# richox/orz

Hardware: AMD Instinct MI355X
Metric: orz -l1 encode throughput (enwik8-shaped text, 100 MB, one 16 MiB block in flight) (higher is better)
Workload: dtype u8

## Files before the change

### orz_amd/csrc/backend_hip.h

```cpp
#pragma once
#include <hip/hip_runtime.h>

#include <cxxabi.h>

#include <chrono>
#include <condition_variable>
#include <algorithm>
#include <atomic>
#include <cstring>
#include <map>
#include <mutex>
#include <rocprim/rocprim.hpp>
#include <stdexcept>
#include <string>
#include <type_traits>
#include <vector>

#include "orz_kernels.h"
#include "orz_parse.h"
#include "orz_symrank.h"

namespace orz {

#define ORZ_HIP_CHECK(expr)                                                                              \
    do {                                                                                                 \
        hipError_t e_ = (expr);                                                                          \
        if (e_ != hipSuccess)                                                                            \
            throw std::runtime_error(std::string("HIP error: ") + hipGetErrorString(e_) + " at " #expr); \
    } while (0)

template <class F>
__global__ __launch_bounds__(256) void orz_thread_kernel(F f, size_t n) {
    size_t tid = (size_t)blockIdx.x * blockDim.x + threadIdx.x;
    if (tid < n) f(tid);
}

#if defined(ORZ_EVAL_WAVES)
template <class F>
__global__ __launch_bounds__(256) __attribute__((amdgpu_waves_per_eu(ORZ_EVAL_WAVES, ORZ_EVAL_WAVES))) void orz_thread_kernel_occ(F f, size_t n) {
    size_t tid = (size_t)blockIdx.x * blockDim.x + threadIdx.x;
    if (tid < n) f(tid);
}
#endif

struct DevWave {
    uint8_t* lds_;
    __device__ __forceinline__ uint32_t lane() const { return threadIdx.x; }
    __device__ __forceinline__ uint32_t block() const { return blockIdx.x; }
    __device__ __forceinline__ uint8_t* lds() const { return lds_; }
    __device__ __forceinline__ uint64_t ballot(bool p) const { return __ballot(p); }
    __device__ __forceinline__ void sync() const { __syncthreads(); }
    __device__ __forceinline__ uint32_t bcast(uint32_t v, uint32_t src) const {
        return (uint32_t)__builtin_amdgcn_readlane((int)v, (int)src);
    }
    __device__ __forceinline__ uint32_t shfl(uint32_t v, uint32_t src) const { return (uint32_t)__shfl((int)v, (int)src, 64); }
    __device__ __forceinline__ uint64_t bcast64(uint64_t v, uint32_t src) const {
        const uint32_t lo = (uint32_t)__builtin_amdgcn_readlane((int)(uint32_t)v, (int)src);
        const uint32_t hi = (uint32_t)__builtin_amdgcn_readlane((int)(uint32_t)(v >> 32), (int)src);
        return (uint64_t)lo | ((uint64_t)hi << 32);
    }
    __device__ __forceinline__ unsigned long long clock() const { return __builtin_amdgcn_s_memtime(); }
    __device__ __forceinline__ unsigned long long wallclock() const { return __builtin_amdgcn_s_memrealtime(); }
};
template <class K>
__global__ __launch_bounds__(64) void orz_wave_kernel(K k) {
    extern __shared__ __attribute__((aligned(16))) uint8_t orz_dyn_lds[];
    DevWave w{orz_dyn_lds};
    k(w);
}

template <class K>
__global__ __launch_bounds__(1024) void orz_group_kernel(K k, bool use_lds) {
    extern __shared__ __attribute__((aligned(16))) uint8_t orz_dyn_lds[];
    for (uint32_t ph = 0; ph < K::kPhases; ph++) {
        if (ph) {
            __threadfence_block();
            __syncthreads();
        }
        k.phase(ph, threadIdx.x, blockDim.x, orz_dyn_lds, use_lds);
    }
}

__global__ __launch_bounds__(256) void orz_rank_kernel(RankArgs a, uint32_t nchunks, uint32_t nvblk) {
    __shared__ uint32_t rows[(kRankChunk + 1) * 256];
    auto sync = [] __device__() { __syncthreads(); };
    if (blockIdx.x < nchunks) rank_chunk(a, blockIdx.x, threadIdx.x, rows, sync);
    else if (blockIdx.x < nchunks + nvblk)
        rebuild_summaries(a.vbits, a.v1, a.v2, a.nvwords, blockIdx.x - nchunks, threadIdx.x, (uint64_t*)rows, sync);
    else
        rebuild_summaries(a.kbits, a.k1, a.k2, a.nkwords, blockIdx.x - nchunks - nvblk, threadIdx.x, (uint64_t*)rows, sync);
}


struct FastEval;

class ParseTokens {
   public:
    static ParseTokens& of(int device) {
        static ParseTokens t[64];
        return t[device & 63];
    }
    void acquire() {
        if (!limit()) return;
        std::unique_lock<std::mutex> lk(m_);
        cv_.wait(lk, [&] { return busy_ < limit(); });
        busy_++;
    }
    void release() {
        if (!limit()) return;
        { std::lock_guard<std::mutex> lk(m_); busy_--; }
        cv_.notify_one();
    }
    static int limit() {
        static const int n = getenv("ORZ_PARSE_TOKENS") ? atoi(getenv("ORZ_PARSE_TOKENS")) : 0;
        return n;
    }

   private:
    std::mutex m_;
    std::condition_variable cv_;
    int busy_ = 0;
// ... 232 lines not shown
    double now() {
        return std::chrono::duration<double>(std::chrono::steady_clock::now().time_since_epoch()).count();
    }
    struct Bracket {
        HipBackend& be;
        bool on;
        Bracket(HipBackend& b, int id) : be(b), on(b.profile_ && !b.capturing_) {
            if (on) be.named_begin(id);
        }
        ~Bracket() {
            if (on) be.named_end();
        }
    };
    template <class F>
    void launch(size_t n, const F& f) {
        if (!n) return;
        Bracket br(*this, profile_ ? KernelNames::of<F>() : 0);
        const unsigned grid = (unsigned)((n + 255) / 256);
#if defined(ORZ_EVAL_WAVES)
        if constexpr (std::is_same<F, FastEval>::value) {
            hipLaunchKernelGGL(orz_thread_kernel_occ<F>, dim3(grid), dim3(256), 0, stream_, f, n);
            ORZ_HIP_CHECK(hipGetLastError());
            return;
        }
#endif
        hipLaunchKernelGGL(orz_thread_kernel<F>, dim3(grid), dim3(256), 0, stream_, f, n);
        ORZ_HIP_CHECK(hipGetLastError());
    }
    template <auto Kernel>
    hipError_t big_lds(int bytes) {
        static std::atomic<int> done[64];
        std::atomic<int>* d = device_ >= 0 && device_ < 64 ? &done[device_] : nullptr;
        if (d) {
            const int v = d->load(std::memory_order_acquire);
            if (v) return (hipError_t)(v - 1);
        }
        int cur = -1;
        ORZ_HIP_CHECK(hipGetDevice(&cur));
        if (cur != device_) ORZ_HIP_CHECK(hipSetDevice(device_));
        const hipError_t e = hipFuncSetAttribute(reinterpret_cast<const void*>(Kernel), hipFuncAttributeMaxDynamicSharedMemorySize, bytes);
        if (cur != device_) ORZ_HIP_CHECK(hipSetDevice(cur));
        if (d) d->store(1 + (int)e, std::memory_order_release);
        return e;
    }
    template <class K>
    void launch_waves(size_t nblocks, const K& k, size_t lds_bytes) {
        if (!nblocks) return;
        Bracket br(*this, profile_ ? KernelNames::of<K>() : 0);
        if (lds_bytes > 64 * 1024) {
            const hipError_t big = big_lds<&orz_wave_kernel<K>>(160 * 1024 - 256);
            if (big != hipSuccess) throw std::runtime_error(std::string("hipFuncSetAttribute(MaxDynamicSharedMemorySize): ") + hipGetErrorString(big));
        }
        hipLaunchKernelGGL(orz_wave_kernel<K>, dim3((unsigned)nblocks), dim3(64), lds_bytes, stream_, k);
        ORZ_HIP_CHECK(hipGetLastError());
    }
    template <class K>
    void launch_group(const K& k) {
        Bracket br(*this, profile_ ? KernelNames::of<K>() : 0);
        size_t lds = k.lds_bytes();
        const bool big_ok = big_lds<&orz_group_kernel<K>>((int)K::kLdsMax) == hipSuccess;
        if (lds > 64 * 1024 && !big_ok) lds = 0;
        hipLaunchKernelGGL(orz_group_kernel<K>, dim3(1), dim3(1024), lds, stream_, k, lds != 0);
        ORZ_HIP_CHECK(hipGetLastError());
    }
    void huffbuild(const HuffBuild& f) {
        if (f.nchunks) launch_waves((size_t)f.nchunks * 3, HuffWave{f}, HuffWave::lds_bytes());
    }
    void rank(const RankArgs& a, uint32_t nchunks) {
        const uint32_t nvblk = (a.nvwords + 4095) / 4096, nkblk = (a.nkwords + 4095) / 4096;
        hipLaunchKernelGGL(orz_rank_kernel, dim3(nchunks + nvblk + nkblk), dim3(256), 0, stream_, a, nchunks, nvblk);
        ORZ_HIP_CHECK(hipGetLastError());
    }
    void sort_pairs_u32(const uint32_t* kin, uint32_t* kout, const uint32_t* vin, uint32_t* vout, size_t n, int bits) {
        if (n == 0) return;
        Bracket br(*this, profile_ ? KernelNames::lib("(radix sort, pairs)") : 0);
        size_t sz = tmp_bytes_;
        ORZ_HIP_CHECK(rocprim::radix_sort_pairs(tmp_, sz, kin, kout, vin, vout, n, 0, (unsigned)bits, stream_));
    }
    void sort_by_ctx(const uint16_t* ctx, uint16_t* ctx_sorted, uint32_t* perm, size_t n) {
        if (n == 0) return;
        Bracket br(*this, profile_ ? KernelNames::lib("(radix sort, items by context)") : 0);
        size_t sz = tmp_bytes_;
        ORZ_HIP_CHECK(rocprim::radix_sort_pairs(tmp_, sz, ctx, ctx_sorted, rocprim::counting_iterator<uint32_t>(0), perm, n, 0, 9, stream_));
    }
    const uint64_t* sort_u64(uint64_t* a, uint64_t* b, size_t n, int bits, int begin_bit = 0) {
        if (n == 0) return a;
        Bracket br(*this, profile_ ? KernelNames::lib("(radix sort, 64-bit keys)") : 0);
        size_t sz = tmp_bytes_;
        ORZ_HIP_CHECK(rocprim::radix_sort_keys(tmp_, sz, a, b, n, (unsigned)begin_bit, (unsigned)bits, stream_));
        return b;
    }
    void exclusive_scan_u32(const uint32_t* in, uint32_t* out, size_t n) {
        if (n == 0) return;
        Bracket br(*this, profile_ ? KernelNames::lib("(scan)") : 0);
        size_t sz = tmp_bytes_;
        ORZ_HIP_CHECK(rocprim::exclusive_scan(tmp_, sz, in, out, 0u, n, rocprim::plus<uint32_t>(), stream_));
    }
    void inclusive_max_scan_u32(const uint32_t* in, uint32_t* out, size_t n) {
        if (n == 0) return;
        Bracket br(*this, profile_ ? KernelNames::lib("(scan, running maximum)") : 0);
        size_t sz = tmp_bytes_;
        ORZ_HIP_CHECK(rocprim::inclusive_scan(tmp_, sz, in, out, n, rocprim::maximum<uint32_t>(), stream_));
    }
    static constexpr int kTimedSlots = 4;
    void timed_begin(int slot = 0) {
        if (!timing_ || capturing_ || ((slot == 0 || slot == 3) && !profile_)) return;
// ... 199 lines not shown
```

### orz_amd/csrc/orz_fast.h

```cpp
#pragma once
#include "orz_kernels.h"
#include "orz_parse.h"

namespace orz {

#if !defined(__HIPCC__)
inline unsigned long long g_far_stats[4] = {0, 0, 0, 0};
#endif

constexpr uint32_t kSub = 4096;
constexpr uint32_t kSeg64 = 64;
constexpr uint32_t kNSub = kNewMax / kSub + 2;
constexpr uint32_t kEntries = 240;

constexpr uint32_t kFastK = 32;
constexpr uint32_t kHistSub = (kPre + 1) / kSub;
constexpr uint32_t kRingMargin = 4;
constexpr uint32_t kFastTile = 262144;
constexpr uint32_t kFastRounds = 4;
constexpr uint32_t kSettledTile = 393216;
constexpr uint32_t kSettledTileDeep = 262144;
constexpr uint32_t kSettledRounds = 3;

struct FastArgs {
// ... 989 lines not shown
                    const uint32_t d = p < a.len ? fast_decide(p, a.len, e[q], e[q + 1], e[q + 2]) : 0;
                    tyw |= (uint64_t)(d & 0xff) << (8 * q);
                    nlw |= (uint64_t)((d >> 8) & 0xff) << (8 * q);
                }
                if ((x >> 10) == part) {
                    if (x + 8 <= clen) {
                        *reinterpret_cast<uint64_t*>(a.ty + i0) = tyw;
                        *reinterpret_cast<uint64_t*>(a.nl + i0) = nlw;
                    } else {
                        for (uint32_t q = 0; x + q < clen; q++) { a.ty[i0 + q] = (uint8_t)(tyw >> (8 * q)); a.nl[i0 + q] = (uint8_t)(nlw >> (8 * q)); }
                    }
                }
            }
            st8_pad68(nlL, x, nlw);
        }
        w.sync();
        {
            const uint32_t s0 = lane * 64;
            if (s0 < clen) {
                const uint32_t s1 = fast_min(s0 + 64, clen), sl = s1 - s0;
                uint32_t adv[16];
                const uint32_t* row = reinterpret_cast<const uint32_t*>(nlL + lane * 68);
#pragma unroll
                for (uint32_t q = 0; q < 16; q++) adv[q] = row[q];
                uint8_t* xrow = x0L + lane * 68;
#pragma unroll
                for (uint32_t k = 0; k < 64; k++) {
                    const uint32_t p = 63 - k;
                    if (p < sl) {
                        const uint32_t d = (adv[p >> 2] >> (8 * (p & 3))) & 0xff, x = p + (d ? d : 1);
                        xrow[p] = x >= sl ? (uint8_t)(x - sl) : xrow[x];
                    }
                }
            }
        }
        w.sync();
        for (uint32_t k = part * 2; k < part * 2 + 2; k++) {
            const uint32_t x = (k * 64 + lane) * 8;
            if (x >= clen) continue;
            const uint32_t* src = reinterpret_cast<const uint32_t*>(x0L + pad68(x));
            *reinterpret_cast<uint64_t*>(a.x0 + (cs - kPre) + x) = (uint64_t)src[0] | ((uint64_t)src[1] << 32);
        }
        w.sync();
        if (lane < 60) {
            const uint32_t e = part * 60 + lane;
            uint32_t x = e;
            while (x < clen) {
                const uint32_t s1 = fast_min(((x >> 6) + 1) * 64, clen);
                x = s1 + x0L[pad68(x)];
            }
            a.x1[(size_t)c * kEntries + e] = (uint8_t)(x - clen);
        }
    }
};
struct PathMarkWave {
    FastArgs a;
    uint32_t c0;
    static constexpr uint32_t kTab = 64 * 68 + 32;
    static size_t lds_bytes() { return 3 * kTab + (65 * 68 + 12) + 256 * 4; }
    template <class W>
    ORZ_D void operator()(W& w) const {
        uint8_t* nlL = w.lds();
        uint8_t* x0L = nlL + kTab;
        uint8_t* tyL = x0L + kTab;
        uint8_t* wL = tyL + kTab;
        uint32_t* cnt = (uint32_t*)(wL + 65 * 68 + 12);
        const uint32_t c = c0 + w.block(), lane = w.lane();
        const uint32_t cs = kPre + c * kSub, clen = chunk_end(c, a.len) - cs;
        for (uint32_t k = lane; k < 256; k += 64) cnt[k] = 0;
        {
            uint64_t v[8], u[8], t[8], b[8];
#pragma unroll
            for (uint32_t k = 0; k < 8; k++) {
                const uint32_t x = (k * 64 + lane) * 8;
                v[k] = u[k] = t[k] = 0;
                if (x < clen) {
                    v[k] = *reinterpret_cast<const uint64_t*>(a.nl + (cs - kPre) + x);
                    u[k] = *reinterpret_cast<const uint64_t*>(a.x0 + (cs - kPre) + x);
                    t[k] = *reinterpret_cast<const uint64_t*>(a.ty + (cs - kPre) + x);
                }
                b[k] = ldu64(a.win + cs - 2 + x);
            }
#pragma unroll
            for (uint32_t k = 0; k < 8; k++) {
                const uint32_t x = (k * 64 + lane) * 8;
                st8_pad68(nlL, x, v[k]); st8_pad68(x0L, x, u[k]); st8_pad68(tyL, x, t[k]);
                st8_pad68(wL, x, b[k]);
            }
        }
        if (lane == 0) st8_pad68(wL, kSub, ldu64(a.win + cs - 2 + kSub));
        w.sync();
        const uint32_t s0 = lane * 64;
        if (s0 < clen) {
            const uint32_t s1 = fast_min(s0 + 64, clen);
            const uint32_t ce = a.centry[c];
            uint32_t x = ce >= cs ? ce - cs : 0;
            while (x < s0) {
                const uint32_t e1 = fast_min(((x >> 6) + 1) * 64, clen);
                x = e1 + x0L[pad68(x)];
            }
            uint64_t m = 0;
            while (x < s1) {
                m |= 1ull << (x - s0);
                atom_add32(&cnt[(uint32_t)(wL[pad68(x + 1)] & 0x7f) | ((uint32_t)is_alnum(wL[pad68(x)]) << 7)], 1);
                const uint32_t d = nlL[pad68(x)];
                const uint32_t e = x + (d ? d : 1);
                a.pt[(cs - kPre) + e] = tyL[pad68(x)];
                x = e;
            }
            a.sbits[(cs - kPre) / 64 + lane] = m;
        }
        w.sync();
        for (uint32_t k = lane; k < 256; k += 64) a.cm[(size_t)c * 256 + k] = cnt[k];
    }
};
ORZ_D uint32_t tile_end(uint32_t t, uint32_t tile, uint32_t len) { return fast_min(len, kPre + (t + 1) * tile); }
struct PathTileDown {
    FastArgs a;
    uint32_t t0, nt;
    static constexpr uint32_t kPhases = 3;
    static constexpr size_t kLdsMax = 144 * 1024;
    ORZ_HD uint32_t range_chunks() const {
        const uint32_t cpt = a.tile / kSub, c0 = t0 * cpt;
        const uint32_t end = kPre + (t0 + nt) * a.tile;
        return ((a.len < end ? a.len : end) - (kPre + c0 * kSub) + kSub - 1) / kSub;
    }
    size_t lds_bytes() const {
        const size_t need = ((size_t)range_chunks() + nt) * kEntries + 16;
        return need <= kLdsMax ? need : 0;
    }
    ORZ_HD void phase(uint32_t ph, uint32_t tid, uint32_t nth, uint8_t* lds, bool use_lds) const {
        const uint32_t cpt = a.tile / kSub, c0 = t0 * cpt, nch = range_chunks();
        uint8_t* x2L = lds + (((size_t)nch * kEntries + 15) & ~(size_t)15);
        const uint8_t* x1p = use_lds ? lds : a.x1 + (size_t)c0 * kEntries;
        uint8_t* x2p = use_lds ? x2L : a.x2 + (size_t)t0 * kEntries;
        if (ph == 0) {
            if (!use_lds) return;
            const uint8_t* src = a.x1 + (size_t)c0 * kEntries;
            struct alignas(16) Q { uint32_t w[4]; };
            const uint32_t nq = nch * kEntries / 16;
            const Q* s16 = reinterpret_cast<const Q*>(src);
            Q* d16 = reinterpret_cast<Q*>(lds);
            for (uint32_t k0 = tid; k0 < nq; k0 += 4 * nth) {
                Q v[4];
#pragma unroll
                for (uint32_t u = 0; u < 4; u++) if (k0 + u * nth < nq) v[u] = s16[k0 + u * nth];
#pragma unroll
                for (uint32_t u = 0; u < 4; u++) if (k0 + u * nth < nq) d16[k0 + u * nth] = v[u];
            }
        } else if (ph == 1) {
            for (uint32_t k = tid; k < nt * kEntries; k += nth) {
                const uint32_t t = t0 + k / kEntries, e = k % kEntries;
                const uint32_t end = tile_end(t, a.tile, a.len);
                uint32_t x = kPre + t * a.tile + e;
                while (x < end) {
                    const uint32_t c = (x - kPre) / kSub;
                    x = chunk_end(c, a.len) + x1p[(size_t)(c - c0) * kEntries + (x - kPre - c * kSub)];
                }
                const uint8_t v = (uint8_t)(x >= end ? x - end : 0);
                a.x2[(size_t)t * kEntries + e] = v;
                if (use_lds) x2p[(size_t)(t - t0) * kEntries + e] = v;
            }
        } else {
            for (uint32_t k = tid; k <= nch; k += nth) {
                const bool tail = k == nch;
                const uint32_t c = c0 + k, t = tail ? t0 + nt : c / cpt;
                uint32_t x = a.tentry[t0];
                for (uint32_t tt = t0; tt < t; tt++) {
                    const uint32_t end = tile_end(tt, a.tile, a.len);
                    if (x < end) x = end + x2p[(size_t)(tt - t0) * kEntries + (x - kPre - tt * a.tile)];
                }
                if (tail) { a.tentry[t] = x; continue; }
                if (c == t * cpt && t > t0) a.tentry[t] = x;
                for (uint32_t cc = t * cpt; cc < c; cc++) {
                    const uint32_t end = chunk_end(cc, a.len);
                    if (x < end) x = end + x1p[(size_t)(cc - c0) * kEntries + (x - kPre - cc * kSub)];
                }
                a.centry[c] = x;
            }
        }
    }
};
struct PathMark {
    FastArgs a;
    uint32_t s0, ns;
    ORZ_HD void operator()(size_t tid) const {
        const uint32_t s = s0 + (uint32_t)tid;
        if (tid >= ns) return;
        const uint32_t start = kPre + s * kSeg64, end = seg_end(s, a.len);
        uint32_t x = a.centry[(start - kPre) / kSub];
        while (x < start) {
            const uint32_t ss = (x - kPre) / kSeg64;
            x = seg_end(ss, a.len) + a.x0[x - kPre];
        }
        uint64_t m = 0;
        while (x < end) {
            m |= 1ull << (x - start);
            const uint32_t d = a.nl[x - kPre];
            const uint32_t e = x + (d ? d : 1);
            a.pt[e - kPre] = a.ty[x - kPre];
            x = e;
        }
        a.sbits[s] = m;
    }
};
struct FastFlip {
    FastArgs a;
    uint32_t lo, hi;
    uint32_t next_entry;
    uint32_t mark_hi;
    uint32_t last_hi;
    uint32_t* lastflips;
    static constexpr uint32_t kTrip = 16;
    ORZ_D uint32_t walk(bool words, uint32_t slot, uint32_t y) const {
        const uint32_t* pos = words ? a.kpos : a.epos;
        const uint64_t* bits = words ? a.kbits : a.vbits;
        const uint32_t lim = words ? 1u : a.dmax;
        const uint32_t end = words ? fast_min(a.nk, slot + 1 + 64) : fast_min(*a.nentp, slot + 1 + kFastK);
        uint32_t passed = 0, n = 0;
        for (uint32_t s = slot + 1; s < end; s += kTrip) {
            if (a.dbg & 64) atom_add64(&a.stats[words ? 19 : 18], 1);
            uint32_t q[kTrip];
#pragma unroll
            for (uint32_t b = 0; b < kTrip; b++) q[b] = s + b < end ? pos[s + b] : 0;
            const uint64_t w0 = racy_load64(&bits[s >> 6]), w1 = racy_load64(&bits[(s + kTrip - 1) >> 6]);
#pragma unroll
            for (uint32_t b = 0; b < kTrip; b++) {
                const uint32_t qq = q[b];
                if (s + b >= end || qq <= y || qq >= mark_hi) return n;
                n++;
// ... 810 lines not shown
```

### orz_amd/csrc/orz_stream.h

```cpp
#pragma once
#include <algorithm>
#include <atomic>
#include <cstdio>
#include <cstdlib>
#include <cstring>
#include <stdexcept>
#include <string>
#include <vector>

#include "orz_fast.h"
#include "orz_kernels.h"
#include "orz_parse.h"
#include "orz_verify.h"

namespace orz {

struct ItemTrace {
    std::vector<uint32_t> block, pos, src;
    std::vector<uint16_t> sym, ctx, rank, rob;
    std::vector<uint8_t> unl, enc, al, mlen;
    void clear() { block.clear(); pos.clear(); src.clear(); sym.clear(); ctx.clear(); rank.clear(); rob.clear(); unl.clear(); enc.clear(); al.clear(); mlen.clear(); }
};

struct FastTableCapture {
    int arm = -1;
    bool taken = false;
    std::vector<std::pair<std::string, std::vector<uint8_t>>> tab;
    const std::vector<uint8_t>* find(const char* name) const {
        for (const auto& t : tab) if (t.first == name) return &t.second;
        return nullptr;
    }
};

struct EncodeStats {
    uint64_t blocks = 0, sweeps = 0, seg_evals = 0, items = 0, chunks = 0, in_bytes = 0, out_bytes = 0;
    uint64_t rank_redos = 0;
    uint64_t host_syncs = 0;
    double t_prep = 0, t_parse = 0, t_post = 0;
};

struct HistFlags32 {
    const uint8_t* S;
    uint32_t* f;
    ORZ_HD void operator()(size_t tid) const {
        if (tid < kPre) f[tid] = (tid >= 1 && S[tid]) ? 1u : 0u;
    }
};
struct Flags32 {
    const uint8_t* S;
    uint32_t n;
    uint32_t* f;
    ORZ_HD void operator()(size_t tid) const {
        if (tid < n) f[tid] = S[kPre + tid];
    }
};
struct SumLast {
    const uint32_t *scan, *flag;
    uint32_t last;
    uint32_t* out;
    ORZ_HD void operator()(size_t tid) const {
// ... 251 lines not shown
    }
};
struct FrameInject {
    uint8_t* dst;
    unsigned long long at;
    ORZ_HD void operator()(size_t tid) const {
        if (tid) return;
        uint64_t tb = 0, lenb = 0, sh = 0;
        for (;;) { const uint8_t b = dst[lenb++]; tb |= (uint64_t)(b & 0x7f) << sh; sh += 7; if (!(b & 0x80)) break; }
        if (at < tb) dst[lenb + at] ^= 1;
    }
};
inline size_t stream_bound(size_t n) { return 2 * n + n / 64 + (1u << 20); }

class ByteBuf {
   public:
    ByteBuf() = default;
    ~ByteBuf() { std::free(p_); }
    ByteBuf(const ByteBuf&) = delete;
    ByteBuf& operator=(const ByteBuf&) = delete;
    void reserve(size_t c) {
        if (c <= cap_) return;
        void* q = std::realloc(p_, c);
        if (!q) throw std::bad_alloc();
        p_ = (uint8_t*)q;
        cap_ = c;
    }
    void resize(size_t m) {
        if (m > cap_) reserve(std::max(m, cap_ * 2));
        n_ = m;
    }
    void push_back(uint8_t b) {
        if (n_ == cap_) reserve(cap_ ? cap_ * 2 : 4096);
        p_[n_++] = b;
    }
    size_t size() const { return n_; }
    bool empty() const { return n_ == 0; }
    uint8_t* data() { return p_; }
    const uint8_t* data() const { return p_; }
    void clear() { n_ = 0; }
    uint8_t* release() {
        if (!p_) reserve(1);
        uint8_t* q = p_;
        p_ = nullptr;
        n_ = cap_ = 0;
        return q;
    }

   private:
    uint8_t* p_ = nullptr;
    size_t n_ = 0, cap_ = 0;
};

template <class BE>
class StreamEncoder {
   public:
    static constexpr size_t kChunkCapWords = (size_t)kChunkItems * 40 / 32 + 8192;
    static constexpr uint32_t kMaxChunks = 17;
    static constexpr uint32_t kNumKeys = 256 * kHash;
    static constexpr uint32_t kDirtyWords = kNumKeys / 64 + 1;
    static constexpr int kFirstPasses = 12;
    static constexpr uint32_t kRepairGrid = 16384;

    StreamEncoder(BE& be, Cfg cfg, uint32_t seg_size = 62, uint32_t win_segs = 3072, bool fast = false,
                  uint32_t fast_tile = kFastTile, uint32_t fast_rounds = kFastRounds)
        : be_(be), cfg_(cfg), seg_(seg_size), wsegs_(win_segs), fast_(fast), ftile_(fast_tile), frounds_(fast_rounds) {
        if (fast_) {
            if (ftile_ < kSub || ftile_ % kSub || ftile_ > kNewMax) throw std::runtime_error("fast tile must be a multiple of 4096 in [4096, 16777216]");
            if (frounds_ < 1 || frounds_ > 64) throw std::runtime_error("fast rounds must be in [1, 64]");
            fK_ = kFastK;
            sched_auto_ = ftile_ == kFastTile && frounds_ == kFastRounds;
            if (cfg.depth > 20) sched_tile_ = kSettledTileDeep;
            if (const char* sc = getenv("ORZ_FAST_SCHED")) {
                unsigned t = 0, r = 0;
                if (sscanf(sc, "%ux%u", &t, &r) == 2 && t >= kSub && t % kSub == 0 && t <= kNewMax && r >= 1 && r <= 64) { sched_tile_ = t; sched_rounds_ = r; }
                else if (!strcmp(sc, "0")) sched_auto_ = false;
                else throw std::runtime_error("ORZ_FAST_SCHED must be 0 or <tile>x<rounds>");
            }
            if (const char* u = getenv("ORZ_FAST_UNIT")) unit_ = (uint32_t)atoi(u);
            if (unit_ < (1u << 20) || unit_ > kNewMax || unit_ % kSub) throw std::runtime_error("ORZ_FAST_UNIT must be a multiple of 4096 in [1 MiB, 16 MiB]");
            cur_unit_ = unit_;
            if (const char* u = getenv("ORZ_FAST_LEADUNIT")) lead_unit_ = (uint32_t)atoi(u);
            if (lead_unit_ && (lead_unit_ < (1u << 20) || lead_unit_ > kNewMax || lead_unit_ % kSub)) throw std::runtime_error("ORZ_FAST_LEADUNIT must be 0 or a multiple of 4096 in [1 MiB, 16 MiB]");
        }
        if (const char* inj = getenv("ORZ_VERIFY_INJECT")) {
            static const char* names[] = {"", "hole", "context", "ring", "lenmin", "word", "bytes", "lenmin2"};
            const std::string v(inj);
            const size_t colon = v.find(':');
            const std::string cls = v.substr(0, colon);
            for (uint32_t k = 1; k < 8; k++)
                if (cls == names[k]) inject_kind_ = k;
            if (!inject_kind_) throw std::runtime_error("ORZ_VERIFY_INJECT: unknown class");
            inject_nth_ = colon == std::string::npos ? 0 : (uint32_t)strtoul(v.c_str() + colon + 1, nullptr, 10);
        }
        if (const char* oi = getenv("ORZ_OUTPUT_INJECT")) out_inject_ = (size_t)strtoull(oi, nullptr, 10);
        for (const char* hook : {"ORZ_VERIFY_INJECT", "ORZ_OUTPUT_INJECT", "ORZ_SYMRANK_INJECT"})
            if (getenv(hook))
                fprintf(stderr, "orz: WARNING: the test hook %s is set in the environment: this encoder DELIBERATELY DAMAGES what it encodes "
                                "(its streams are invalid unless a guard catches the damage); unset it for real use\n", hook);
        if (seg_ < 8 || seg_ > kSegMax) throw std::runtime_error("seg_size must be in [8, 62]");
        if (wsegs_ < 1) throw std::runtime_error("window must hold at least one segment");
        try {
            dmax_ = (uint32_t)std::max(cfg.depth, std::max(cfg.lazy1, cfg.lazy2));
            if (cfg.depth < 1 || dmax_ > 200) throw std::runtime_error("LZCfg depth out of range");
            nseg_max_ = (kNewMax + seg_ - 1) / seg_;
            if (wsegs_ > nseg_max_) wsegs_ = nseg_max_;
            ring_ = wsegs_ + 8;
            winbuf_ = take<uint8_t>((size_t)kBlock + 2 * kSent + 64);
            S_ = take<uint8_t>(kWLen);
            if (!fast_) E_ = take<uint8_t>(kWLen);
            ML_ = take<uint8_t>(kWLen);
            ORD_ = take<uint32_t>(kWLen);
            if (!fast_) LR_ = take<uint8_t>(kWLen);
            SRC_ = take<uint32_t>(kWLen, false);
            W0_ = take<uint8_t>(kWLen);
            TY_ = take<uint8_t>(kWLen);
            LENMIN_ = take<uint8_t>(kWLen);
            LMV_ = take<uint8_t>(kWLen);
            idx_ = take<uint32_t>(kWLen, false);
            kidx_ = take<uint32_t>(kWLen, false);
            entA_ = take<uint64_t>((size_t)kWLen, false);
            entB_ = take<uint64_t>((size_t)kWLen, false);
            epos_ = take<uint32_t>(kWLen, false);
            kpos_ = take<uint32_t>((size_t)kNewMax + 8);
            runstart_ = take<uint32_t>(kNumKeys + 1);
            krun_ = take<uint32_t>(32768 + 1);
            krunend_ = take<uint32_t>(32768 + 1);
            vbits_ = take<uint64_t>(kWLen / 64 + 2);
            v1_ = take<uint64_t>(kWLen / 4096 + 2);
            v2_ = take<uint64_t>(kWLen / 262144 + 2);
            kbits_ = take<uint64_t>(kNewMax / 64 + 2);
            k1_ = take<uint64_t>(kNewMax / 4096 + 2);
            k2_ = take<uint64_t>(kNewMax / 262144 + 2);
            if (!fast_) {
                srec_ = take<SlotRec>(kWLen);
                exitst_ = take<uint64_t>((size_t)nseg_max_ + 2);
// ... 447 lines not shown
        a.extra = getenv("ORZ_FAST_EXTRA") ? (uint32_t)atoi(getenv("ORZ_FAST_EXTRA")) : (a.depth + 1) / (a.depth < 10 ? 3 : 2);
        a.centry = fcentry_; a.tentry = ftentry_; a.cm = fcm_; a.cp = fcp_; a.nchg = &fctl_->chg; a.nentp = &fctl_->nent;
        be_.launch(1, FastSetNent{fctl_, nent});
        a.dbg = getenv("ORZ_FAST_DBG") ? (uint32_t)atoi(getenv("ORZ_FAST_DBG")) : 0;
        a.stats = fdiag_;
        if (a.dbg & 64) be_.memset(a.stats, 0, 32 * 8);
        uint32_t T = ftile_, R = frounds_;
        bool settled = false;
        {
            static const uint32_t tdiv = getenv("ORZ_FAST_TDIV") ? (uint32_t)atoi(getenv("ORZ_FAST_TDIV")) : 128;
            const uint32_t want = ((n / tdiv + kSub - 1) / kSub) * kSub;
            T = std::max<uint32_t>(kSub, std::min<uint32_t>(ftile_, want));
            const bool big_part = !stream_start_ && n >= cur_unit_ / 2;
            if (n >= cur_unit_ || big_part) T = ftile_;
            static const uint32_t lead_mul = getenv("ORZ_FAST_LEADMUL") ? (uint32_t)atoi(getenv("ORZ_FAST_LEADMUL")) : 1;
            if (lead_block_ && T == ftile_ && lead_mul >= 1 && lead_mul <= 8) T = (uint32_t)std::min<uint64_t>((uint64_t)lead_mul * ftile_, kNewMax);
            if (sched_auto_ && settled_next_ && (n >= cur_unit_ || big_part) && T == ftile_) { T = sched_tile_; R = sched_rounds_; settled = true; }
        }
        for (int attempt = 0;; attempt++) {
            a.tile = T;
            a.rounds = R;
            if (attempt) {
                be_.memset(vbits_ + nent / 64, 0, 16);
                be_.launch_waves(((size_t)nent + 63) / 64, FastSlotInitWave{epos_, nullptr, runstart_, nent, vbits_, frlen_}, 0);
                be_.memset(fccnt_, 0, (size_t)(kNumKeys + 1) * 4);
                be_.launch(nent, FastListReset{epos_, slot_keys, runstart_, nent, fccnt_});
            }
            const size_t nn = (size_t)n + 264;
            {
                ZeroRanges z;
                z.add(kbits_, ((size_t)n / 64 + 2) * 8);
                z.add(k1_, ((size_t)kNewMax / 4096 + 2) * 8);
                z.add(fty_, nn); z.add(fnl_, nn); z.add(fpt_, nn); z.add(fmf_, nn); z.add(fef_, nn);
                z.add(fsbits_, ((size_t)n / 64 + 8) * 8);
                z.add(fcm_, (size_t)(nsub + 2) * 256 * 4);
                z.add(fcp_, (size_t)(nsub + 2) * 256 * 4);
                z.add(&fctl_->lastflips, 4);
                z.add(fcnew_, (size_t)(kNumKeys + 1) * 4);
                if (repair_lists) {
                    z.add(tbits, tbits_bytes);
                    z.add(kdirty, kdirty_bytes);
                    z.add(fcok_, 256 * 4);
                    z.add(frdirty_ + kDirtyWords, (size_t)kDirtyWords * 8);
                }
                be_.launch(z.units(), z);
            }
            be_.launch(nvw / 64 + 1, V1Build{vbits_, nvw, v1_});
            be_.launch(256, FastCpInit{ctxcount_, fcp_, ftentry_});
            const uint32_t ntile = (n + T - 1) / T, cpt = T / kSub;
            be_.launch_waves(256, FastPrefix{a, 0, 0, std::min(cpt + 1, nsub), cpt, 0}, 0);
            { const FastHorizon fh{a, 0, std::min(cpt + 1, nsub) - 1}; be_.launch(fh.threads(), fh); }
            static const bool fused_steps = !(getenv("ORZ_FAST_FUSED") && !strcmp(getenv("ORZ_FAST_FUSED"), "0"));
            const bool use_graph = be_.graphs_enabled() && (n == kNewMax || n == cur_unit_);
            const uint64_t gkey = ((uint64_t)R << 58) | ((uint64_t)T << 32) | n;
            const bool replayed = use_graph && be_.graph_replay(gkey);
            struct CaptureGuard {
                BE& be;
                bool on;
                ~CaptureGuard() { if (on) be.graph_capture_abort(); }
            } capture{be_, use_graph && !replayed};
            if (capture.on) be_.graph_capture_begin();
            if (replayed) stats.sweeps += ntile + R - 1;
            for (uint32_t step = 1; step <= ntile + R - 1 && !replayed; step++) {
                const uint32_t t_lo = step > R ? step - R : 0, t_hi = std::min(step - 1, ntile - 1);
                const uint32_t lo = kPre + t_lo * T;
                const uint32_t hi = (uint32_t)std::min<uint64_t>(len, (uint64_t)kPre + (uint64_t)(t_hi + 1) * T);
                const uint32_t hi2 = std::min(len, hi + 2);
                be_.timed_begin();
                const uint32_t r1lo = step <= ntile ? kPre + t_hi * T : hi;
                const uint32_t r2lo = step >= 2 && step - 2 < ntile ? kPre + (step - 2) * T : (step < 2 ? kPre : hi);
                const uint32_t mark_hi = step - 1 < ntile ? kPre + (step - 1) * T : len;
                const uint32_t cline = kPre + (step > R ? step - R : 0) * T;
                be_.launch(hi2 - lo, FastEval{a, lo, hi2, r1lo, r2lo, step, cline});
                be_.timed_end();
                const uint32_t c0 = t_lo * cpt, nc = (hi - (kPre + c0 * kSub) + kSub - 1) / kSub, nt = t_hi - t_lo + 1;
                be_.timed_begin(3);
                if (fused_steps) {
                    const bool had_retire = step - 1 >= R && step - 1 < ntile + R - 1;
                    const uint32_t plo = had_retire ? kPre + (step - 1 - R) * T : kPre, phi = had_retire ? (uint32_t)std::min<uint64_t>(len, (uint64_t)plo + T) : kPre;
                    PathUpWave up{a, c0};
                    up.decide = 1; up.nup = nc * 4; up.done = FastRetireDone{a, plo, phi, fcut_};
                    be_.launch_waves((size_t)nc * 4 + (phi - plo + 63) / 64, up, PathUpWave::lds_bytes());
                } else {
                    be_.launch(hi - lo, FastDecide{a, lo, hi});
                    be_.launch_waves((size_t)nc * 4, PathUpWave{a, c0}, PathUpWave::lds_bytes());
                }
                be_.timed_end(3);
                be_.launch_group(PathTileDown{a, t_lo, nt});
                be_.launch_waves(nc, PathMarkWave{a, c0}, PathMarkWave::lds_bytes());
                const uint32_t fhi = std::min(len, hi + 240);
                const FastFlip ff{a, lo, fhi, t_hi + 1, mark_hi, step >= R ? (uint32_t)std::min<uint64_t>(len, (uint64_t)lo + T) : 0, &fctl_->lastflips};
                const uint32_t ext = std::min(cpt + 1, nsub - std::min(nsub, c0 + nc));
                const FastPrefix fp{a, c0, c0 + nc, ext, cpt, step >= R ? std::min(c0 + cpt, c0 + nc) : c0};
                const FastHorizon fh{a, c0, c0 + nc + ext - 1};
                const bool retire = step >= R && step < ntile + R - 1;
                const uint32_t rlo = retire ? kPre + (step - R) * T : kPre, rhi = retire ? (uint32_t)std::min<uint64_t>(len, (uint64_t)rlo + T) : kPre;
                if (fused_steps) {
                    const uint32_t nflip = fhi - lo + 1, nret = rhi - rlo;
                    be_.launch_waves(flip_blocks(nflip) + 256, FlipPrefixWave{ff, fp, nflip}, FlipPrefixWave::lds_bytes());
                    be_.launch_waves((size_t)(nret + 63) / 64 + (fh.threads() + 63) / 64, RetireHorizonWave{FastRetire{a, rlo, rhi, fcut_}, fh, nret}, 0);
                } else {
                    be_.launch((size_t)fhi - lo + 1, ff);
                    be_.launch_waves(256, fp, 0);
                    be_.launch(fh.threads(), fh);
                    if (retire) {
                        be_.launch(rhi - rlo, FastRetire{a, rlo, rhi, fcut_});
                        be_.launch(rhi - rlo, FastRetireDone{a, rlo, rhi, fcut_});
                    }
                }
                stats.sweeps++;
            }
            const bool incr_repairs = !getenv("ORZ_FAST_FULLPASS");
            const uint32_t src_cap = getenv("ORZ_FAST_SRCCAP") ? (uint32_t)atoi(getenv("ORZ_FAST_SRCCAP")) : 4 * a.depth + 4;
            static const bool ord_ballots = !(getenv("ORZ_FAST_ORD") && !strcmp(getenv("ORZ_FAST_ORD"), "table"));
            const FastFlip flip_all{a, kPre, len, ~0u, 0, 0, &fctl_->lastflips};
            const uint32_t tw = n / 64 + 1;
            int pass = 0;
            auto lists_pass = [&]() {
                    if (pass == 0) be_.launch((size_t)n + 1, flip_all);
                    else be_.launch(tw, FastFlipSparse{flip_all, tw, kdirty, fctl_});
                    uint64_t* rd_in = frdirty_ + (size_t)(pass & 1) * kDirtyWords;
                    uint64_t* rd_out = frdirty_ + (size_t)((pass + 1) & 1) * kDirtyWords;
                    {
                        FastCokGrow cg{fcok_, fcok_ + 256};
                        cg.ctl = fctl_;
                        if (pass) { cg.rd_out = rd_out; cg.nwords = kDirtyWords; }
                        be_.launch(cg.threads(), cg);
                    }
                    be_.launch_waves(nsub, RepairListWave{a, mlist, wlist, mcnt, wcnt, pass && incr_repairs ? rd_in : nullptr, fdirty_, fcok_ + 256, fctl_},
                                     RepairListWave::lds_bytes());
                    col_scan(fcm_, nsub, fcp_, fctl_);
                    be_.launch(256, FastItemTotal{fcp_, nsub, fctl_});
                    if (ord_ballots) be_.launch_waves(nsub, OrdWave2{win, fsbits_, fcp_, n, ORD_, fctl_}, OrdWave2::lds_bytes());
                    else be_.launch_waves(nsub, OrdWave{win, fsbits_, fcp_, n, ORD_, fctl_}, OrdWave::lds_bytes());
                    FastSource fs{a, SRC_, fcut_, pass && incr_repairs ? rd_in : nullptr, src_cap, fctl_, fdirty_, fcok_ + 256};
                    fs.cutlist = cutlist; fs.ncut = &fctl_->ncut;
                    const uint32_t per = kListThreads;
                    be_.launch((size_t)nsub * per, FastSourceL{fs, mlist, mcnt, nsub, per});
// ... 516 lines not shown
    struct MainStreamGuard {
        BE& be;
        ~MainStreamGuard() { be.select(0); }
    };
    TailSet ts_[2];
    static constexpr uint32_t kTailItems0 = 6u << 20;
    struct Fresh {
        BE& be;
        std::vector<void*> ptrs;
        bool keep = false;
        ~Fresh() {
            if (!keep) for (void* q : ptrs) if (q) be.free(q);
        }
        template <class T>
        T* get(size_t n, bool zero) {
            ptrs.reserve(ptrs.size() + 1);
            T* q = be.template alloc<T>(n, zero);
            ptrs.push_back(q);
            return q;
        }
    };
    void grow_tail_set(TailSet& t, uint32_t need) {
        uint64_t cap = std::max<uint64_t>(need, (uint64_t)t.cap * 3 / 2);
        cap = std::min<uint64_t>(kNewMax, (cap + 65535) & ~65535ull);
        Fresh fresh{be_, {}};
        TailSet nt = t;
        nt.ipos = fresh.template get<uint32_t>((size_t)cap + 1, false);
        nt.isym = fresh.template get<uint16_t>(cap, true); nt.ictx = fresh.template get<uint16_t>(cap, true);
        nt.irank = fresh.template get<uint16_t>(cap, true); nt.irob = fresh.template get<uint16_t>(cap, true);
        nt.grank = fresh.template get<uint16_t>(cap, true); nt.skey = fresh.template get<uint16_t>(cap, true);
        nt.iunl = fresh.template get<uint8_t>(cap, true); nt.ienc = fresh.template get<uint8_t>(cap, true); nt.ial = fresh.template get<uint8_t>(cap, true);
        nt.gsym = fresh.template get<uint32_t>(cap, false); nt.sperm = fresh.template get<uint32_t>(cap, false);
        nt.blen = fresh.template get<uint32_t>(cap, false); nt.bscan = fresh.template get<uint32_t>(cap, false);
        owned_.reserve(owned_.size() + fresh.ptrs.size());
        fresh.keep = true;
        if (t.cap) be_.sync();
        void* old[] = {t.ipos, t.isym, t.ictx, t.irank, t.irob, t.grank, t.skey, t.iunl, t.ienc, t.ial, t.gsym, t.sperm, t.blen, t.bscan};
        for (void* q : old) {
            if (!q) continue;
            be_.free(q);
            owned_.erase(std::find(owned_.begin(), owned_.end(), q));
        }
        for (void* q : fresh.ptrs) owned_.push_back(q);
        nt.cap = (uint32_t)cap;
        t = nt;
    }
    int cur_set_ = 0;
    uint32_t last_n_ = kNewMax;
    uint32_t hist_hint_ = ~0u;
    uint32_t unit_base_ = 0;
    uint32_t unit_ = kNewMax / 2;
    uint32_t cur_unit_ = kNewMax;
    uint32_t lead_unit_ = 0;
    std::vector<int> pend_order_;
    uint8_t* winbuf_;
    uint8_t *S_, *E_ = nullptr, *ML_, *LR_ = nullptr, *W0_, *TY_, *LENMIN_, *LMV_;
    uint32_t *ORD_, *SRC_;
    uint32_t *idx_, *kidx_, *epos_, *kpos_, *runstart_, *krun_, *krunend_;
    uint64_t *entA_, *entB_, *vbits_, *v1_, *v2_, *kbits_, *k1_, *k2_;
    SlotRec* srec_ = nullptr;
    uint64_t* exitst_ = nullptr;
    uint8_t* hist_ = nullptr;
    uint32_t* base_ = nullptr;
    ParseCtl* ctl_ = nullptr;
    uint32_t* partial_ = nullptr;
    uint32_t *f32_, *sc32_, *hpos_, *ctxcount_, *tailkey_;
    uint8_t* wsnap_;
    uint32_t* wlast_;
    uint32_t* counts_;
    uint16_t* order_;
    uint32_t* ncounted_;
    uint16_t* srstate_;
    uint32_t *vrec_ = nullptr, *vord_ = nullptr, *vctx_ = nullptr, *vlast_ = nullptr;
    uint8_t* vwords_ = nullptr;
    uint32_t inject_kind_ = 0, inject_nth_ = 0;
    size_t out_inject_ = 0;
    uint16_t* srbackup_ = nullptr;
    uint64_t* outoff_;
    bool dev_out_ = false;
    uint8_t* dout_ = nullptr;
    uint8_t* own_out_ = nullptr;
    size_t own_cap_ = 0;
    OutCtl* octl_ = nullptr;
    OutCtl hctl_{};
};

template <class BE, class OutT>
void encode_stream(StreamEncoder<BE>& enc, BE& be, const uint8_t* src, size_t n, bool src_on_device,
                   OutT& out, bool src_pinned = false) {
    enc.reset();
    size_t off = 0;
    while (off < n) {
        uint32_t take = (uint32_t)std::min<size_t>(n - off, kNewMax);
        if (src_on_device) be.d2d(enc.dwin() + kPre, src + off, take);
        else if (src_pinned) be.h2d_pinned(enc.dwin() + kPre, src + off, take);
        else be.h2d(enc.dwin() + kPre, src + off, take);
        enc.encode_block_units(take, off == 0 && n > enc.unit_bytes(), out);
        off += take;
        if (off < n) enc.slide();
    }
    enc.finish(out);
    out.push_back(0);
    enc.stats.out_bytes = out.size();
}

template <class BE>
// ... 20 lines not shown
```

Measured before the change: 495.9.

## Run PathUp as 256-thread workgroups and add run-level jump tables to PathTileDown

Adds a workgroup launch path that processes one 4 KiB chunk per 256-thread group, replacing four separate 64-lane wave blocks per chunk. This keeps the decide, segment-jump and chunk-exit steps of a chunk in one group's shared LDS. PathTileDown gains two phases that compose chunk exit tables into 8-chunk run tables, so tile and chunk entry resolution hops over runs instead of walking every chunk serially. It also hardens the LDS copy loads. The group path is on by default, can be switched off with an env var, and uses more LDS and extra barriers.

```diff
diff --git a/orz_amd/csrc/backend_hip.h b/orz_amd/csrc/backend_hip.h
--- a/orz_amd/csrc/backend_hip.h
+++ b/orz_amd/csrc/backend_hip.h
@@ -67,6 +67,22 @@
     extern __shared__ __attribute__((aligned(16))) uint8_t orz_dyn_lds[];
     DevWave w{orz_dyn_lds};
     k(w);
+}
+
+struct DevGroup {
+    uint8_t* lds_;
+    __device__ __forceinline__ uint32_t lane() const { return threadIdx.x & 63; }
+    __device__ __forceinline__ uint32_t wave() const { return threadIdx.x >> 6; }
+    __device__ __forceinline__ uint32_t thread() const { return threadIdx.x; }
+    __device__ __forceinline__ uint32_t block() const { return blockIdx.x; }
+    __device__ __forceinline__ uint8_t* lds() const { return lds_; }
+    __device__ __forceinline__ void sync() const { __syncthreads(); }
+};
+template <class K>
+__global__ __launch_bounds__(256) void orz_wgroup_kernel(K k) {
+    extern __shared__ __attribute__((aligned(16))) uint8_t orz_dyn_lds[];
+    DevGroup g{orz_dyn_lds};
+    k.group(g);
 }
 
 template <class K>
@@ -405,6 +421,18 @@
             if (big != hipSuccess) throw std::runtime_error(std::string("hipFuncSetAttribute(MaxDynamicSharedMemorySize): ") + hipGetErrorString(big));
         }
         hipLaunchKernelGGL(orz_wave_kernel<K>, dim3((unsigned)nblocks), dim3(64), lds_bytes, stream_, k);
+        ORZ_HIP_CHECK(hipGetLastError());
+    }
+    static constexpr bool kHasGroups = true;
+    template <class K>
+    void launch_groups(size_t ngroups, const K& k, size_t lds_bytes) {
+        if (!ngroups) return;
+        Bracket br(*this, profile_ ? KernelNames::of<K>() : 0);
+        if (lds_bytes > 64 * 1024) {
+            const hipError_t big = big_lds<&orz_wgroup_kernel<K>>(160 * 1024 - 256);
+            if (big != hipSuccess) throw std::runtime_error(std::string("hipFuncSetAttribute(MaxDynamicSharedMemorySize): ") + hipGetErrorString(big));
+        }
+        hipLaunchKernelGGL(orz_wgroup_kernel<K>, dim3((unsigned)ngroups), dim3(256), lds_bytes, stream_, k);
         ORZ_HIP_CHECK(hipGetLastError());
     }
     template <class K>
diff --git a/orz_amd/csrc/orz_fast.h b/orz_amd/csrc/orz_fast.h
--- a/orz_amd/csrc/orz_fast.h
+++ b/orz_amd/csrc/orz_fast.h
@@ -1065,6 +1065,96 @@
             a.x1[(size_t)c * kEntries + e] = (uint8_t)(x - clen);
         }
     }
+    template <class G>
+    ORZ_D void group(G& g) const {
+        if (decide && g.block() >= nup) {
+            done((size_t)(g.block() - nup) * 256 + g.thread());
+            return;
+        }
+        uint8_t* nlL = g.lds();
+        uint8_t* x0L = nlL + 64 * 68 + 32;
+        const uint32_t c = c0 + g.block(), part = g.wave(), lane = g.lane();
+        const uint32_t cs = kPre + c * kSub, clen = chunk_end(c, a.len) - cs;
+        uint64_t w5[2][5];
+        if (decide) {
+#pragma unroll
+            for (uint32_t k = 0; k < 2; k++) {
+                const uint32_t x = ((part * 2 + k) * 64 + lane) * 8;
+                const uint64_t* ew = reinterpret_cast<const uint64_t*>(a.ev + (cs - kPre) + (x < clen ? x : 0));
+#pragma unroll
+                for (uint32_t q = 0; q < 5; q++) w5[k][q] = ew[q];
+            }
+        }
+#pragma unroll
+        for (uint32_t k = 0; k < 2; k++) {
+            const uint32_t x = ((part * 2 + k) * 64 + lane) * 8;
+            if (!decide) {
+                st8_pad68(nlL, x, x < clen ? *reinterpret_cast<const uint64_t*>(a.nl + (cs - kPre) + x) : 0);
+                continue;
+            }
+            uint64_t nlw = 0, tyw = 0;
+            if (x < clen) {
+                const uint32_t i0 = (cs - kPre) + x;
+                uint32_t e[10];
+#pragma unroll
+                for (uint32_t q = 0; q < 10; q++) {
+                    const uint32_t v = (uint32_t)(w5[k][q >> 1] >> (32 * (q & 1)));
+                    e[q] = cs + x + q < a.len ? v : 0;
+                }
+#pragma unroll
+                for (uint32_t q = 0; q < 8; q++) {
+                    const uint32_t p = cs + x + q;
+                    const uint32_t d = p < a.len ? fast_decide(p, a.len, e[q], e[q + 1], e[q + 2]) : 0;
+                    tyw |= (uint64_t)(d & 0xff) << (8 * q);
+                    nlw |= (uint64_t)((d >> 8) & 0xff) << (8 * q);
+                }
+                if (x + 8 <= clen) {
+                    *reinterpret_cast<uint64_t*>(a.ty + i0) = tyw;
+                    *reinterpret_cast<uint64_t*>(a.nl + i0) = nlw;
+                } else {
+                    for (uint32_t q = 0; x + q < clen; q++) { a.ty[i0 + q] = (uint8_t)(tyw >> (8 * q)); a.nl[i0 + q] = (uint8_t)(nlw >> (8 * q)); }
+                }
+            }
+            st8_pad68(nlL, x, nlw);
+        }
+        g.sync();
+        {
+            const uint32_t seg = part * 16 + lane, s0 = seg * 64;
+            if (lane < 16 && s0 < clen) {
+                const uint32_t s1 = fast_min(s0 + 64, clen), sl = s1 - s0;
+                uint32_t adv[16];
+                const uint32_t* row = reinterpret_cast<const uint32_t*>(nlL + seg * 68);
+#pragma unroll
+                for (uint32_t q = 0; q < 16; q++) adv[q] = row[q];
+                uint8_t* xrow = x0L + seg * 68;
+#pragma unroll
+                for (uint32_t k = 0; k < 64; k++) {
+                    const uint32_t p = 63 - k;
+                    if (p < sl) {
+                        const uint32_t d = (adv[p >> 2] >> (8 * (p & 3))) & 0xff, x = p + (d ? d : 1);
+                        xrow[p] = x >= sl ? (uint8_t)(x - sl) : xrow[x];
+                    }
+                }
+            }
+        }
+        g.sync();
+#pragma unroll
+        for (uint32_t k = 0; k < 2; k++) {
+            const uint32_t x = ((part * 2 + k) * 64 + lane) * 8;
+            if (x >= clen) continue;
+            const uint32_t* src = reinterpret_cast<const uint32_t*>(x0L + pad68(x));
+            *reinterpret_cast<uint64_t*>(a.x0 + (cs - kPre) + x) = (uint64_t)src[0] | ((uint64_t)src[1] << 32);
+        }
+        if (lane < 60) {
+            const uint32_t e = part * 60 + lane;
+            uint32_t x = e;
+            while (x < clen) {
+                const uint32_t s1 = fast_min(((x >> 6) + 1) * 64, clen);
+                x = s1 + x0L[pad68(x)];
+            }
+            a.x1[(size_t)c * kEntries + e] = (uint8_t)(x - clen);
+        }
+    }
 };
 struct PathMarkWave {
     FastArgs a;
@@ -1131,64 +1221,138 @@
 struct PathTileDown {
     FastArgs a;
     uint32_t t0, nt;
-    static constexpr uint32_t kPhases = 3;
+    static constexpr uint32_t kPhases = 5;
+    static constexpr uint32_t kRun = 8;
     static constexpr size_t kLdsMax = 144 * 1024;
     ORZ_HD uint32_t range_chunks() const {
         const uint32_t cpt = a.tile / kSub, c0 = t0 * cpt;
         const uint32_t end = kPre + (t0 + nt) * a.tile;
         return ((a.len < end ? a.len : end) - (kPre + c0 * kSub) + kSub - 1) / kSub;
     }
+    ORZ_HD uint32_t runs_per_tile() const { return (a.tile / kSub + kRun - 1) / kRun; }
     size_t lds_bytes() const {
-        const size_t need = ((size_t)range_chunks() + nt) * kEntries + 16;
+        const size_t nruns = (size_t)nt * runs_per_tile();
+        const size_t need = ((size_t)range_chunks() + nt + nruns) * kEntries + (nruns + 1) * 4 + 16;
         return need <= kLdsMax ? need : 0;
     }
+    ORZ_HD uint32_t hop_chunk(const uint8_t* x1p, uint32_t c0, uint32_t cc, uint32_t x) const {
+        const uint32_t end = chunk_end(cc, a.len);
+        return x < end ? end + x1p[(size_t)(cc - c0) * kEntries + (x - kPre - cc * kSub)] : x;
+    }
+    ORZ_HD uint32_t hop_run(const uint8_t* yrow, uint32_t ca, uint32_t cb, uint32_t x) const {
+        const uint32_t end = chunk_end(cb - 1, a.len);
+        return x < end ? end + yrow[x - kPre - ca * kSub] : x;
+    }
     ORZ_HD void phase(uint32_t ph, uint32_t tid, uint32_t nth, uint8_t* lds, bool use_lds) const {
-        const uint32_t cpt = a.tile / kSub, c0 = t0 * cpt, nch = range_chunks();
-        uint8_t* x2L = lds + (((size_t)nch * kEntries + 15) & ~(size_t)15);
-        const uint8_t* x1p = use_lds ? lds : a.x1 + (size_t)c0 * kEntries;
-        uint8_t* x2p = use_lds ? x2L : a.x2 + (size_t)t0 * kEntries;
+        const uint32_t cpt = a.tile / kSub, c0 = t0 * cpt, nch = range_chunks(), cN = c0 + nch;
+        if (!use_lds) {
+            const uint8_t* x1p = a.x1 + (size_t)c0 * kEntries;
+            if (ph == 1) {
+                for (uint32_t k = tid; k < nt * kEntries; k += nth) {
+                    const uint32_t t = t0 + k / kEntries, e = k % kEntries;
+                    const uint32_t end = tile_end(t, a.tile, a.len);
+                    uint32_t x = kPre + t * a.tile + e;
+                    while (x < end) x = hop_chunk(x1p, c0, (x - kPre) / kSub, x);
+                    a.x2[(size_t)t * kEntries + e] = (uint8_t)(x >= end ? x - end : 0);
+                }
+            } else if (ph == 2) {
+                for (uint32_t k = tid; k <= nch; k += nth) {
+                    const bool tail = k == nch;
+                    const uint32_t c = c0 + k, t = tail ? t0 + nt : c / cpt;
+                    uint32_t x = a.tentry[t0];
+                    for (uint32_t tt = t0; tt < t; tt++) {
+                        const uint32_t end = tile_end(tt, a.tile, a.len);
+                        if (x < end) x = end + a.x2[(size_t)tt * kEntries + (x - kPre - tt * a.tile)];
+                    }
+                    if (tail) { a.tentry[t] = x; continue; }
+                    if (c == t * cpt && t > t0) a.tentry[t] = x;
+                    for (uint32_t cc = t * cpt; cc < c; cc++) x = hop_chunk(x1p, c0, cc, x);
+                    a.centry[c] = x;
+                }
+            }
+            return;
+        }
+        const uint32_t rpt = runs_per_tile(), nruns = nt * rpt;
+        const uint8_t* x1L = lds;
+        uint8_t* x2L = lds + (size_t)nch * kEntries;
+        uint8_t* yL = x2L + (size_t)nt * kEntries;
+        uint32_t* reL = reinterpret_cast<uint32_t*>(yL + (size_t)nruns * kEntries);
+        auto run_lo = [&](uint32_t t, uint32_t j) { return t * cpt + j * kRun; };
+        auto run_hi = [&](uint32_t t, uint32_t j) { return fast_min(fast_min(t * cpt + (j + 1) * kRun, (t + 1) * cpt), cN); };
         if (ph == 0) {
-            if (!use_lds) return;
             const uint8_t* src = a.x1 + (size_t)c0 * kEntries;
             struct alignas(16) Q { uint32_t w[4]; };
             const uint32_t nq = nch * kEntries / 16;
             const Q* s16 = reinterpret_cast<const Q*>(src);
             Q* d16 = reinterpret_cast<Q*>(lds);
             for (uint32_t k0 = tid; k0 < nq; k0 += 4 * nth) {
-                Q v[4];
-#pragma unroll
-                for (uint32_t u = 0; u < 4; u++) if (k0 + u * nth < nq) v[u] = s16[k0 + u * nth];
-#pragma unroll
-                for (uint32_t u = 0; u < 4; u++) if (k0 + u * nth < nq) d16[k0 + u * nth] = v[u];
+                const Q v0 = s16[k0], v1 = s16[fast_min(k0 + nth, nq - 1)], v2 = s16[fast_min(k0 + 2 * nth, nq - 1)], v3 = s16[fast_min(k0 + 3 * nth, nq - 1)];
+                d16[k0] = v0;
+                if (k0 + nth < nq) d16[k0 + nth] = v1;
+                if (k0 + 2 * nth < nq) d16[k0 + 2 * nth] = v2;
+                if (k0 + 3 * nth < nq) d16[k0 + 3 * nth] = v3;
             }
         } else if (ph == 1) {
+            const uint32_t n = nruns * kEntries;
+            for (uint32_t k0 = tid; k0 < n; k0 += 4 * nth) {
+                uint32_t x[4], ca[4], cb[4];
+#pragma unroll
+                for (uint32_t u = 0; u < 4; u++) {
+                    const uint32_t k = k0 + u * nth, r = (k < n ? k : 0) / kEntries, e = k % kEntries;
+                    const uint32_t t = t0 + r / rpt, j = r % rpt;
+                    ca[u] = run_lo(t, j);
+                    cb[u] = k < n ? run_hi(t, j) : 0;
+                    x[u] = kPre + ca[u] * kSub + e;
+                }
+                for (uint32_t h = 0; h < kRun; h++) {
+                    uint32_t idx[4], end[4];
+                    uint8_t v[4];
+#pragma unroll
+                    for (uint32_t u = 0; u < 4; u++) {
+                        const uint32_t cc = ca[u] + h;
+                        end[u] = cc < cb[u] ? chunk_end(cc, a.len) : 0;
+                        idx[u] = x[u] < end[u] ? (cc - c0) * kEntries + (x[u] - kPre - cc * kSub) : 0;
+                    }
+#pragma unroll
+                    for (uint32_t u = 0; u < 4; u++) v[u] = x1L[idx[u]];
+#pragma unroll
+                    for (uint32_t u = 0; u < 4; u++) x[u] = x[u] < end[u] ? end[u] + v[u] : x[u];
+                }
+#pragma unroll
+                for (uint32_t u = 0; u < 4; u++)
+                    if (ca[u] < cb[u]) yL[k0 + u * nth] = (uint8_t)(x[u] - chunk_end(cb[u] - 1, a.len));
+            }
+        } else if (ph == 2) {
             for (uint32_t k = tid; k < nt * kEntries; k += nth) {
                 const uint32_t t = t0 + k / kEntries, e = k % kEntries;
                 const uint32_t end = tile_end(t, a.tile, a.len);
                 uint32_t x = kPre + t * a.tile + e;
-                while (x < end) {
-                    const uint32_t c = (x - kPre) / kSub;
-                    x = chunk_end(c, a.len) + x1p[(size_t)(c - c0) * kEntries + (x - kPre - c * kSub)];
-                }
+                for (uint32_t j = 0; j < rpt && run_lo(t, j) < cN; j++)
+                    x = hop_run(yL + (size_t)((t - t0) * rpt + j) * kEntries, run_lo(t, j), run_hi(t, j), x);
                 const uint8_t v = (uint8_t)(x >= end ? x - end : 0);
                 a.x2[(size_t)t * kEntries + e] = v;
-                if (use_lds) x2p[(size_t)(t - t0) * kEntries + e] = v;
-            }
-        } else {
-            for (uint32_t k = tid; k <= nch; k += nth) {
-                const bool tail = k == nch;
-                const uint32_t c = c0 + k, t = tail ? t0 + nt : c / cpt;
+                x2L[(size_t)(t - t0) * kEntries + e] = v;
+            }
+        } else if (ph == 3) {
+            for (uint32_t r = tid; r <= nruns; r += nth) {
+                const bool tail = r == nruns;
+                const uint32_t t = tail ? t0 + nt : t0 + r / rpt, j = tail ? 0 : r % rpt;
                 uint32_t x = a.tentry[t0];
                 for (uint32_t tt = t0; tt < t; tt++) {
                     const uint32_t end = tile_end(tt, a.tile, a.len);
-                    if (x < end) x = end + x2p[(size_t)(tt - t0) * kEntries + (x - kPre - tt * a.tile)];
+                    if (x < end) x = end + x2L[(size_t)(tt - t0) * kEntries + (x - kPre - tt * a.tile)];
                 }
                 if (tail) { a.tentry[t] = x; continue; }
-                if (c == t * cpt && t > t0) a.tentry[t] = x;
-                for (uint32_t cc = t * cpt; cc < c; cc++) {
-                    const uint32_t end = chunk_end(cc, a.len);
-                    if (x < end) x = end + x1p[(size_t)(cc - c0) * kEntries + (x - kPre - cc * kSub)];
-                }
+                if (j == 0 && t > t0) a.tentry[t] = x;
+                for (uint32_t jj = 0; jj < j && run_lo(t, jj) < cN; jj++)
+                    x = hop_run(yL + (size_t)((t - t0) * rpt + jj) * kEntries, run_lo(t, jj), run_hi(t, jj), x);
+                reL[r] = x;
+            }
+        } else {
+            for (uint32_t k = tid; k < nch; k += nth) {
+                const uint32_t c = c0 + k, t = c / cpt, j = (c - t * cpt) / kRun;
+                uint32_t x = reL[(t - t0) * rpt + j];
+                for (uint32_t cc = run_lo(t, j); cc < c; cc++) x = hop_chunk(x1L, c0, cc, x);
                 a.centry[c] = x;
             }
         }
diff --git a/orz_amd/csrc/orz_stream.h b/orz_amd/csrc/orz_stream.h
--- a/orz_amd/csrc/orz_stream.h
+++ b/orz_amd/csrc/orz_stream.h
@@ -6,6 +6,7 @@
 #include <cstring>
 #include <stdexcept>
 #include <string>
+#include <type_traits>
 #include <vector>
 
 #include "orz_fast.h"
@@ -363,6 +364,11 @@
     size_t n_ = 0, cap_ = 0;
 };
 
+template <class BE, class = void>
+struct has_groups : std::false_type {};
+template <class BE>
+struct has_groups<BE, std::enable_if_t<BE::kHasGroups>> : std::true_type {};
+
 template <class BE>
 class StreamEncoder {
    public:
@@ -393,6 +399,10 @@
             cur_unit_ = unit_;
             if (const char* u = getenv("ORZ_FAST_LEADUNIT")) lead_unit_ = (uint32_t)atoi(u);
             if (lead_unit_ && (lead_unit_ < (1u << 20) || lead_unit_ > kNewMax || lead_unit_ % kSub)) throw std::runtime_error("ORZ_FAST_LEADUNIT must be 0 or a multiple of 4096 in [1 MiB, 16 MiB]");
+            if (const char* pu = getenv("ORZ_FAST_PATHUP")) {
+                if (!strcmp(pu, "waves")) pathup_group_ = false;
+                else if (strcmp(pu, "group")) throw std::runtime_error("ORZ_FAST_PATHUP must be waves or group");
+            }
         }
         if (const char* inj = getenv("ORZ_VERIFY_INJECT")) {
             static const char* names[] = {"", "hole", "context", "ring", "lenmin", "word", "bytes", "lenmin2"};
@@ -946,7 +956,9 @@
             { const FastHorizon fh{a, 0, std::min(cpt + 1, nsub) - 1}; be_.launch(fh.threads(), fh); }
             static const bool fused_steps = !(getenv("ORZ_FAST_FUSED") && !strcmp(getenv("ORZ_FAST_FUSED"), "0"));
             const bool use_graph = be_.graphs_enabled() && (n == kNewMax || n == cur_unit_);
-            const uint64_t gkey = ((uint64_t)R << 58) | ((uint64_t)T << 32) | n;
+            bool up_group = false;
+            if constexpr (has_groups<BE>::value) up_group = pathup_group_;
+            const uint64_t gkey = ((uint64_t)R << 58) | ((uint64_t)up_group << 57) | ((uint64_t)T << 32) | n;
             const bool replayed = use_graph && be_.graph_replay(gkey);
             struct CaptureGuard {
                 BE& be;
@@ -973,11 +985,27 @@
                     const bool had_retire = step - 1 >= R && step - 1 < ntile + R - 1;
                     const uint32_t plo = had_retire ? kPre + (step - 1 - R) * T : kPre, phi = had_retire ? (uint32_t)std::min<uint64_t>(len, (uint64_t)plo + T) : kPre;
                     PathUpWave up{a, c0};
-                    up.decide = 1; up.nup = nc * 4; up.done = FastRetireDone{a, plo, phi, fcut_};
-                    be_.launch_waves((size_t)nc * 4 + (phi - plo + 63) / 64, up, PathUpWave::lds_bytes());
+                    up.decide = 1; up.done = FastRetireDone{a, plo, phi, fcut_};
+                    if constexpr (has_groups<BE>::value) {
+                        if (up_group) {
+                            up.nup = nc;
+                            be_.launch_groups((size_t)nc + (phi - plo + 255) / 256, up, PathUpWave::lds_bytes());
+                        }
+                    }
+                    if (!up_group) {
+                        up.nup = nc * 4;
+                        be_.launch_waves((size_t)nc * 4 + (phi - plo + 63) / 64, up, PathUpWave::lds_bytes());
+                    }
                 } else {
                     be_.launch(hi - lo, FastDecide{a, lo, hi});
-                    be_.launch_waves((size_t)nc * 4, PathUpWave{a, c0}, PathUpWave::lds_bytes());
+                    PathUpWave up{a, c0};
+                    if constexpr (has_groups<BE>::value) {
+                        if (up_group) {
+                            up.nup = nc;
+                            be_.launch_groups(nc, up, PathUpWave::lds_bytes());
+                        }
+                    }
+                    if (!up_group) be_.launch_waves((size_t)nc * 4, up, PathUpWave::lds_bytes());
                 }
                 be_.timed_end(3);
                 be_.launch_group(PathTileDown{a, t_lo, nt});
@@ -1600,6 +1628,7 @@
     uint32_t unit_ = kNewMax / 2;
     uint32_t cur_unit_ = kNewMax;
     uint32_t lead_unit_ = 0;
+    bool pathup_group_ = true;
     std::vector<int> pend_order_;
     uint8_t* winbuf_;
     uint8_t *S_, *E_ = nullptr, *ML_, *LR_ = nullptr, *W0_, *TY_, *LENMIN_, *LMV_;
```

Result: no change. 500.6, median of 3 (+0.9%).
